# crisbodnar/text-to-image

Measured on AMD Instinct MI355X. Metric: images/sec (G+D step) at 64x64 batch=64, higher is better.
Workload: dtype f32; 1 GPU; wgancls 64x64 batch=64/GPU fp32, synthetic images + random 1024-d text embeddings, D step (+kt) then G step, Adam(b1=0,b2=0.9); global_batch=64, parallelism=dp1, launch=hipGraph replay (1 graph/iteration)

## Files before the change

text-to-image_amd/csrc/t2i_bgemm.hip:

```cpp
#include <hip/hip_runtime.h>
#include <stdint.h>

#include <type_traits>

#include "t2i_internal.h"

namespace t2i {

typedef float f32x16 __attribute__((ext_vector_type(16)));
typedef unsigned int u32x4 __attribute__((ext_vector_type(4)));

namespace {
constexpr int BK = 32;
constexpr int KSTRIDE = BK + 4;
constexpr unsigned OOB = 0xFFFFFFF0u;

template <int LAY, int WM, int WN, int NW = 4>
struct BSmem {
  static constexpr bool A_KIN = LAY != 2, B_KIN = LAY == 1;
  static constexpr int BM = 32 * (NW / 2) * WM, BN = 64 * WN;
  static constexpr int A_ELEMS = A_KIN ? BM * KSTRIDE : BK * BM;
  static constexpr int B_ELEMS = B_KIN ? BN * KSTRIDE : BK * BN;
  static constexpr int BYTES = 2 * (A_ELEMS + B_ELEMS) * 4;
};
// ... 86 lines not shown
      }
    }
  };

  float4 areg[A_LD], breg[B_LD];
  auto load_into = [&](float4* ar, float4* br) __attribute__((always_inline)) {
    const int k0 = l_t * BK;
    ++l_t;
#pragma unroll
    for (int i = 0; i < A_LD; ++i) {
      if (A_KIN) ar[i] = bl4(ra, a_off[i] + k0, a_ok[i] & (k0 + kq * 4 < p.K));
      else ar[i] = bl4(ra, a_off[i] + k0 * p.M, a_ok[i] & (k0 + a_kr + A_KR * i < p.K));
    }
#pragma unroll
    for (int i = 0; i < B_LD; ++i) {
      if (B_KIN) br[i] = bl4(rb, b_off[i] + k0, b_ok[i] & (k0 + kq * 4 < p.K));
      else br[i] = bl4(rb, b_off[i] + k0 * p.N, b_ok[i] & (k0 + b_kr + B_KR * i < p.K));
    }
  };
  auto load_tile = [&]() __attribute__((always_inline)) { load_into(areg, breg); };
  auto store_from = [&](int buf, const float4* ar, const float4* br) __attribute__((always_inline)) {
    float* as = As + buf * S::A_ELEMS;
    float* bs = Bs + buf * S::B_ELEMS;
#pragma unroll
    for (int i = 0; i < A_LD; ++i) {
      if (A_KIN) *reinterpret_cast<float4*>(&as[(r0 + RPP * i) * KSTRIDE + kq * 4]) = ar[i];
      else *reinterpret_cast<float4*>(&as[(a_kr + A_KR * i) * BM + a_c4 * 4]) = ar[i];
    }
#pragma unroll
    for (int i = 0; i < B_LD; ++i) {
      if (B_KIN) *reinterpret_cast<float4*>(&bs[(r0 + RPP * i) * KSTRIDE + kq * 4]) = br[i];
      else *reinterpret_cast<float4*>(&bs[(b_kr + B_KR * i) * BN + b_c4 * 4]) = br[i];
    }
  };
  auto store_tile = [&](int buf) __attribute__((always_inline)) { store_from(buf, areg, breg); };

  struct Frag { float a[WM][4]; float b[WN][4]; };
  auto read_frag = [&](Frag& f, const float* as, const float* bs, int c) __attribute__((always_inline)) {
#pragma unroll
    for (int i = 0; i < WM; ++i) {
      const int row = (wm * WM + i) * 32 + l31;
      if (A_KIN) {
        const float4 v = *reinterpret_cast<const float4*>(&as[row * KSTRIDE + c * 8 + lh * 4]);
        f.a[i][0] = v.x; f.a[i][1] = v.y; f.a[i][2] = v.z; f.a[i][3] = v.w;
      } else {
#pragma unroll
        for (int j = 0; j < 4; ++j) f.a[i][j] = as[(c * 8 + j + 4 * lh) * BM + row];
      }
    }
#pragma unroll
    for (int i = 0; i < WN; ++i) {
      const int col = (wn * WN + i) * 32 + l31;
      if (B_KIN) {
        const float4 v = *reinterpret_cast<const float4*>(&bs[col * KSTRIDE + c * 8 + lh * 4]);
        f.b[i][0] = v.x; f.b[i][1] = v.y; f.b[i][2] = v.z; f.b[i][3] = v.w;
      } else {
#pragma unroll
        for (int j = 0; j < 4; ++j) f.b[i][j] = bs[(c * 8 + j + 4 * lh) * BN + col];
      }
    }
  };

  f32x16 acc[WM][WN];
#pragma unroll
  for (int i = 0; i < WM; ++i)
#pragma unroll
    for (int n = 0; n < WN; ++n)
#pragma unroll
      for (int e = 0; e < 16; ++e) acc[i][n][e] = 0.f;
  auto mma_frag = [&](const Frag& f) __attribute__((always_inline)) {
#pragma unroll
    for (int j = 0; j < 4; ++j)
#pragma unroll
      for (int i = 0; i < WM; ++i)
#pragma unroll
        for (int n = 0; n < WN; ++n)
          acc[i][n] = __builtin_amdgcn_mfma_f32_32x32x2f32(f.a[i][j], f.b[n][j], acc[i][n], 0, 0, 0);
  };
  constexpr int N_MMA = 4 * WM * WN, N_PIECE = A_LD + B_LD, MMA_PER_PIECE = N_MMA / N_PIECE > 0 ? N_MMA / N_PIECE : 1;

  auto k_tile = [&](int t, Frag& c0, Frag& c1, Frag& n0, Frag& n1) __attribute__((always_inline)) {
    const float* as = As + (t & 1) * S::A_ELEMS;
    const float* bs = Bs + (t & 1) * S::B_ELEMS;
    const float* an = As + ((t + 1) & 1) * S::A_ELEMS;
    const float* bn_ = Bs + ((t + 1) & 1) * S::B_ELEMS;
    __builtin_amdgcn_sched_barrier(0);
    mma_frag(c0);
    __builtin_amdgcn_sched_barrier(0);
    read_frag(c0, as, bs, 2);
    __builtin_amdgcn_sched_barrier(0);
    mma_frag(c1);
    store_tile((t + 1) & 1);
#pragma unroll
    for (int q2 = 0; q2 < N_PIECE; ++q2) {
      __builtin_amdgcn_sched_group_barrier(0x008, MMA_PER_PIECE, 0);
      __builtin_amdgcn_sched_group_barrier(0x200, 1, 0);
    }
    __builtin_amdgcn_sched_barrier(0);
    read_frag(c1, as, bs, 3);
    __builtin_amdgcn_sched_barrier(0);
    __syncthreads();
    read_frag(n0, an, bn_, 0);
    read_frag(n1, an, bn_, 1);
    __builtin_amdgcn_sched_barrier(0);
    load_tile();
    mma_frag(c0);
#pragma unroll
    for (int q2 = 0; q2 < N_PIECE; ++q2) {
      __builtin_amdgcn_sched_group_barrier(0x008, MMA_PER_PIECE, 0);
      __builtin_amdgcn_sched_group_barrier(0x020, 1, 0);
    }
    __builtin_amdgcn_sched_barrier(0);
    mma_frag(c1);
  };

  next_item();
  {
    float4 a0[A_LD], b0[B_LD];
    load_into(a0, b0);
    load_tile();
    store_from(0, a0, b0);
  }
  __syncthreads();
  Frag fa0, fa1, fb0, fb1;
  read_frag(fa0, As, Bs, 0);
  read_frag(fa1, As, Bs, 1);
  for (int it = 0; it < n_items; ++it) {
    for (int t = 0; t < p.ntiles; t += 2) {
      if (t + 2 == p.ntiles) next_item();
      k_tile(0, fa0, fa1, fb0, fb1);
      k_tile(1, fb0, fb1, fa0, fa1);
    }
    int bz, bm, bn;
    coords(run0 + slot + it * nslot, bz, bm, bn);
    float* out = p.c + (int64_t)bz * p.sc;
#pragma unroll
    for (int i = 0; i < WM; ++i)
#pragma unroll
      for (int j = 0; j < WN; ++j) {
        const int n = bn + (wn * WN + j) * 32 + l31;
#pragma unroll
        for (int e = 0; e < 16; ++e) {
          const int m = bm + (wm * WM + i) * 32 + (e & 3) + 8 * (e >> 2) + 4 * lh;
          if (m < p.M && n < p.N) out[(size_t)m * p.N + n] = acc[i][j][e];
        }
#pragma unroll
        for (int e = 0; e < 16; ++e) acc[i][j][e] = 0.f;
      }
  }
}

template <int LAY, bool XF = false>
__global__ __launch_bounds__(256, 2) void bgemm9_kernel(Bgemm9Params q) {
  static_assert(!XF || LAY == 1, "the in-loader input transform exists for the input-gradient form");
  const BgemmParams& p = q.g;
  using S = BSmem<LAY, 1, 1, 4>;
  constexpr bool B_KIN = S::B_KIN;
  constexpr int BM = 64, BN = 64, A_LD = 2, B_LD = 2;
  constexpr int B_C4 = BN / 4, B_KR = 256 / B_C4;
  extern __shared__ __attribute__((aligned(16))) float smem_b[];
  float* As = smem_b;
  float* Bs = smem_b + 2 * S::A_ELEMS;

  const int tid = threadIdx.x;
  const int lane = tid & 63, wave = tid >> 6;
  const int wm = wave >> 1, wn = wave & 1;
  const int l31 = lane & 31, lh = lane >> 5;

  const int nslot = gridDim.x >> 3;
  const int xcd = blockIdx.x & 7, slot = blockIdx.x >> 3;
  const int qq = p.items >> 3, rr_ = p.items & 7;
  const int run0 = xcd * qq + min(xcd, rr_), runlen = qq + (xcd < rr_ ? 1 : 0);
  if (slot >= runlen) return;
  const int n_items = (runlen - slot + nslot - 1) / nslot;
  const int tiles = p.tiles_m * p.tiles_n;

  auto coords = [&](int w, int& phs, int& bm, int& bn) __attribute__((always_inline)) {
    phs = w / tiles;
    const int t = w - phs * tiles;
    const int g = p.group_n, per_group = g * p.tiles_m;
    const int grp = t / per_group, rr = t - grp * per_group, n0 = grp * g;
    const int width = min(g, p.tiles_n - n0);
    const int tm = rr / width;
    bm = tm * BM;
    bn = (n0 + rr - tm * width) * BN;
  };
  auto plane_slot = [&](int pos, int phs) __attribute__((always_inline)) {
    if (LAY == 0) return pos;
    const int r = pos / 3, c = pos - 3 * r;
    return ((2 - r) * 3 + (2 - c)) * 4 + (3 - phs);
  };

  const int kq = tid & 7, r0 = tid >> 3;
  const int b_c4 = tid % B_C4, b_kr = tid / B_C4;
  __amdgpu_buffer_rsrc_t ra, rb;
  int a_off[A_LD], b_off[B_LD];
  bool a_ok[A_LD], b_ok[B_LD];
  unsigned a_win[A_LD];
  int x_tap[4];
  unsigned x_bit[4];
  int l_item = -1, l_pos = 8, l_t = 0, l_phs = 0, l_bm = 0, l_bn = 0;
  if (XF) ra = __builtin_amdgcn_make_buffer_rsrc(const_cast<float*>(q.dy), (short)0, (int)p.a_bytes, 0x00020000);

  auto next_sub = [&]() __attribute__((always_inline)) {
    l_t = 0;
    bool new_item = false;
    if (++l_pos == 9) {
      l_pos = 0;
      ++l_item;
      new_item = true;
      if (l_item < n_items) coords(run0 + slot + l_item * nslot, l_phs, l_bm, l_bn);
    }
    if (l_item >= n_items) {
#pragma unroll
      for (int i = 0; i < A_LD; ++i) { a_ok[i] = false; a_win[i] = 0u; }
#pragma unroll
      for (int i = 0; i < B_LD; ++i) b_ok[i] = false;
      return;
    }
    const int ps = plane_slot(l_pos, l_phs);
    if (!XF) ra = __builtin_amdgcn_make_buffer_rsrc(const_cast<float*>(p.a + (int64_t)ps * p.sa), (short)0, (int)p.a_bytes, 0x00020000);
    rb = __builtin_amdgcn_make_buffer_rsrc(const_cast<float*>(p.b + (int64_t)ps * p.sb), (short)0, (int)p.b_bytes, 0x00020000);
    if (XF) {
      const int r = l_pos / 3, c = l_pos - 3 * r;
      const int rowpx = q.dWo * p.K;
      x_tap[0] = r * rowpx + c * p.K;  x_bit[0] = 1u << (r * 3 + c);
      x_tap[1] = 1 * rowpx + c * p.K;  x_bit[1] = r != 1 ? 1u << (3 + c) : 0u;
      x_tap[2] = r * rowpx + 1 * p.K;  x_bit[2] = c != 1 ? 1u << (r * 3 + 1) : 0u;
      x_tap[3] = 1 * rowpx + 1 * p.K;  x_bit[3] = (r != 1 && c != 1) ? 1u << 4 : 0u;
      if (new_item) {
        const int ph = l_phs >> 1, pw = l_phs & 1;
#pragma unroll
        for (int i = 0; i < A_LD; ++i) {
          const int m = l_bm + r0 + 32 * i;
          const int b = m / (q.Th * q.Tw), rem = m - b * (q.Th * q.Tw);
          const int ty = rem / q.Tw, tx = rem - ty * q.Tw;
          const int oh0 = 2 * ty + ph - 1, ow0 = 2 * tx + pw - 1;
          a_off[i] = ((b * q.dHo + oh0) * q.dWo + ow0) * p.K + kq * 4;
          unsigned w = 0u;
#pragma unroll
          for (int rr2 = 0; rr2 < 3; ++rr2)
#pragma unroll
            for (int cc2 = 0; cc2 < 3; ++cc2)
              if ((unsigned)(oh0 + rr2) < (unsigned)q.dHo && (unsigned)(ow0 + cc2) < (unsigned)q.dWo) w |= 1u << (rr2 * 3 + cc2);
          a_win[i] = m < p.M ? w : 0u;
        }
      }
    } else {
#pragma unroll
      for (int i = 0; i < A_LD; ++i) {
        const int m = l_bm + r0 + 32 * i;
        a_ok[i] = m < p.M;
        a_off[i] = m * p.K + kq * 4;
      }
    }
#pragma unroll
    for (int i = 0; i < B_LD; ++i) {
      if (B_KIN) {
        const int n = l_bn + r0 + 32 * i;
        b_ok[i] = n < p.N;
        b_off[i] = n * p.K + kq * 4;
      } else {
        const int n = l_bn + b_c4 * 4;
        b_ok[i] = n < p.N;
        b_off[i] = (b_kr + B_KR * i) * p.N + n;
      }
    }
  };

  float4 areg[A_LD], breg[B_LD];
  auto load_into = [&](float4* ar, float4* br) __attribute__((always_inline)) {
    const int k0 = l_t * BK;
    ++l_t;
    if (XF) {
      const bool kin = k0 + kq * 4 < p.K;
#pragma unroll
      for (int i = 0; i < A_LD; ++i) {
        const float4 ta = bl4(ra, a_off[i] + x_tap[0] + k0, kin & ((a_win[i] & x_bit[0]) != 0u));
        const float4 tb = bl4(ra, a_off[i] + x_tap[1] + k0, kin & ((a_win[i] & x_bit[1]) != 0u));
        const float4 tc = bl4(ra, a_off[i] + x_tap[2] + k0, kin & ((a_win[i] & x_bit[2]) != 0u));
        const float4 td = bl4(ra, a_off[i] + x_tap[3] + k0, kin & ((a_win[i] & x_bit[3]) != 0u));
        ar[i] = make_float4((ta.x - tb.x) - (tc.x - td.x), (ta.y - tb.y) - (tc.y - td.y), (ta.z - tb.z) - (tc.z - td.z), (ta.w - tb.w) - (tc.w - td.w));
      }
    } else {
#pragma unroll
      for (int i = 0; i < A_LD; ++i) ar[i] = bl4(ra, a_off[i] + k0, a_ok[i] & (k0 + kq * 4 < p.K));
    }
#pragma unroll
    for (int i = 0; i < B_LD; ++i) {
      if (B_KIN) br[i] = bl4(rb, b_off[i] + k0, b_ok[i] & (k0 + kq * 4 < p.K));
      else br[i] = bl4(rb, b_off[i] + k0 * p.N, b_ok[i] & (k0 + b_kr + B_KR * i < p.K));
    }
  };
  auto store_from = [&](int buf, const float4* ar, const float4* br) __attribute__((always_inline)) {
    float* as = As + buf * S::A_ELEMS;
    float* bs = Bs + buf * S::B_ELEMS;
#pragma unroll
    for (int i = 0; i < A_LD; ++i) *reinterpret_cast<float4*>(&as[(r0 + 32 * i) * KSTRIDE + kq * 4]) = ar[i];
#pragma unroll
    for (int i = 0; i < B_LD; ++i) {
      if (B_KIN) *reinterpret_cast<float4*>(&bs[(r0 + 32 * i) * KSTRIDE + kq * 4]) = br[i];
      else *reinterpret_cast<float4*>(&bs[(b_kr + B_KR * i) * BN + b_c4 * 4]) = br[i];
    }
  };

  struct Frag { float a[4]; float b[4]; };
  auto read_frag = [&](Frag& f, const float* as, const float* bs, int c) __attribute__((always_inline)) {
    {
      const int row = wm * 32 + l31;
      const float4 v = *reinterpret_cast<const float4*>(&as[row * KSTRIDE + c * 8 + lh * 4]);
      f.a[0] = v.x; f.a[1] = v.y; f.a[2] = v.z; f.a[3] = v.w;
    }
    {
      const int col = wn * 32 + l31;
      if (B_KIN) {
        const float4 v = *reinterpret_cast<const float4*>(&bs[col * KSTRIDE + c * 8 + lh * 4]);
        f.b[0] = v.x; f.b[1] = v.y; f.b[2] = v.z; f.b[3] = v.w;
      } else {
#pragma unroll
        for (int j = 0; j < 4; ++j) f.b[j] = bs[(c * 8 + j + 4 * lh) * BN + col];
      }
    }
  };

  f32x16 acc[9];
#pragma unroll
  for (int i = 0; i < 9; ++i)
#pragma unroll
    for (int e = 0; e < 16; ++e) acc[i][e] = 0.f;

  auto k_tile = [&](auto P_, int t, Frag& c0, Frag& c1, Frag& n0, Frag& n1) __attribute__((always_inline)) {
    constexpr int P = decltype(P_)::value;
    const float* as = As + (t & 1) * S::A_ELEMS;
    const float* bs = Bs + (t & 1) * S::B_ELEMS;
    const float* an = As + ((t + 1) & 1) * S::A_ELEMS;
    const float* bn_ = Bs + ((t + 1) & 1) * S::B_ELEMS;
    auto mma = [&](const Frag& f) __attribute__((always_inline)) {
#pragma unroll
      for (int j = 0; j < 4; ++j) acc[P] = __builtin_amdgcn_mfma_f32_32x32x2f32(f.a[j], f.b[j], acc[P], 0, 0, 0);
    };
    __builtin_amdgcn_sched_barrier(0);
    mma(c0);
    __builtin_amdgcn_sched_barrier(0);
    read_frag(c0, as, bs, 2);
    __builtin_amdgcn_sched_barrier(0);
    mma(c1);
    store_from((t + 1) & 1, areg, breg);
#pragma unroll
    for (int q2 = 0; q2 < 4; ++q2) {
      __builtin_amdgcn_sched_group_barrier(0x008, 1, 0);
      __builtin_amdgcn_sched_group_barrier(0x200, 1, 0);
    }
    __builtin_amdgcn_sched_barrier(0);
    read_frag(c1, as, bs, 3);
    __builtin_amdgcn_sched_barrier(0);
    __syncthreads();
    read_frag(n0, an, bn_, 0);
    read_frag(n1, an, bn_, 1);
    __builtin_amdgcn_sched_barrier(0);
    load_into(areg, breg);
    mma(c0);
#pragma unroll
    for (int q2 = 0; q2 < 4; ++q2) {
      __builtin_amdgcn_sched_group_barrier(0x008, 1, 0);
      __builtin_amdgcn_sched_group_barrier(0x020, 1, 0);
    }
    __builtin_amdgcn_sched_barrier(0);
    mma(c1);
  };

  next_sub();
  {
    float4 a0[A_LD], b0[B_LD];
    load_into(a0, b0);
    load_into(areg, breg);
    store_from(0, a0, b0);
  }
  __syncthreads();
  Frag fa0, fa1, fb0, fb1;
  read_frag(fa0, As, Bs, 0);
  read_frag(fa1, As, Bs, 1);
  auto run_pos = [&](auto P_) __attribute__((always_inline)) {
    for (int t = 0; t < p.ntiles; t += 2) {
      if (t + 2 == p.ntiles) next_sub();
      k_tile(P_, 0, fa0, fa1, fb0, fb1);
      k_tile(P_, 1, fb0, fb1, fa0, fa1);
    }
  };
  const int plane_px = q.Th * q.Tw;
  for (int it = 0; it < n_items; ++it) {
    run_pos(std::integral_constant<int, 0>{}); run_pos(std::integral_constant<int, 1>{}); run_pos(std::integral_constant<int, 2>{});
    run_pos(std::integral_constant<int, 3>{}); run_pos(std::integral_constant<int, 4>{}); run_pos(std::integral_constant<int, 5>{});
    run_pos(std::integral_constant<int, 6>{}); run_pos(std::integral_constant<int, 7>{}); run_pos(std::integral_constant<int, 8>{});
    int phs, bm, bn;
    coords(run0 + slot + it * nslot, phs, bm, bn);
    const int ph = phs >> 1, pw = phs & 1;
    const int n = bn + wn * 32 + l31;
    const float bs_ = (q.bias && n < p.N) ? q.bias[n] : 0.f;
#pragma unroll
    for (int e = 0; e < 16; ++e) {
      const int m = bm + wm * 32 + (e & 3) + 8 * (e >> 2) + 4 * lh;
      float z[2][3];
#pragma unroll
      for (int c = 0; c < 3; ++c) {
        z[0][c] = acc[0 * 3 + c][e] + acc[1 * 3 + c][e];
        z[1][c] = acc[1 * 3 + c][e] + acc[2 * 3 + c][e];
      }
      if (m < p.M && n < p.N) {
        const int b = m / plane_px, rem = m - b * plane_px;
        const int ty = rem / q.Tw, tx = rem - ty * q.Tw;
#pragma unroll
        for (int r = 0; r < 2; ++r) {
          const float y0 = apply_act((z[r][0] + z[r][1]) + bs_, q.act, q.alpha);
          const float y1 = apply_act((z[r][1] + z[r][2]) + bs_, q.act, q.alpha);
          const size_t oh = (size_t)q.sr * (2 * ty + r) + ph, ow0 = (size_t)q.sr * (2 * tx) + pw;
          float* o = q.out + (((size_t)b * q.OH + oh) * q.OW + ow0) * p.N + n;
          o[0] = y0;
          o[(size_t)q.sr * p.N] = y1;
        }
      }
    }
#pragma unroll
    for (int i = 0; i < 9; ++i)
#pragma unroll
      for (int e = 0; e < 16; ++e) acc[i][e] = 0.f;
  }
}

hipError_t bgemm9_launch(int lay, const Bgemm9Params& q, hipStream_t stream) {
  if (lay != 0 && lay != 1) return hipErrorInvalidValue;
  const int bytes = lay == 0 ? BSmem<0, 1, 1, 4>::BYTES : BSmem<1, 1, 1, 4>::BYTES;
  const int per_xcd = (q.g.items + 7) / 8;
  int nslot = per_xcd < 32 * 2 ? per_xcd : 32 * 2;
  if (nslot < 1) nslot = 1;
  if (lay == 0) hipLaunchKernelGGL((bgemm9_kernel<0, false>), dim3(nslot * 8), dim3(256), bytes, stream, q);
  else if (q.dy) hipLaunchKernelGGL((bgemm9_kernel<1, true>), dim3(nslot * 8), dim3(256), bytes, stream, q);
  else hipLaunchKernelGGL((bgemm9_kernel<1, false>), dim3(nslot * 8), dim3(256), bytes, stream, q);
  return hipGetLastError();
}

template <int LAY, int WM, int WN, int NW = 4>
static hipError_t launch_b(const BgemmParams& p, hipStream_t stream) {
  using S = BSmem<LAY, WM, WN, NW>;
  auto k = bgemm_kernel<LAY, WM, WN, NW>;
  static bool attr_done = false;
  if (!attr_done && S::BYTES > 48 * 1024) {
    hipError_t e = hipFuncSetAttribute(reinterpret_cast<const void*>(k), hipFuncAttributeMaxDynamicSharedMemorySize, S::BYTES);
    if (e != hipSuccess) return e;
    attr_done = true;
  }
  const int per_cu = (WM * WN == 1 && NW == 4) ? 4 : 2;
  const int per_xcd = (p.items + 7) / 8;
  int nslot = per_xcd < 32 * per_cu ? per_xcd : 32 * per_cu;
  if (nslot < 1) nslot = 1;
  hipLaunchKernelGGL(k, dim3(nslot * 8), dim3(64 * NW), S::BYTES, stream, p);
  return hipGetLastError();
}

hipError_t bgemm_launch(int lay, int wm, int wn, const BgemmParams& p, hipStream_t stream) {
  if (wm == 4 && wn == 1) {
    if (lay == 0) return launch_b<0, 1, 1, 8>(p, stream);
    if (lay == 1) return launch_b<1, 1, 1, 8>(p, stream);
    if (lay == 2) return launch_b<2, 1, 1, 8>(p, stream);
  }
#define T2I_B(L, a, b) if (lay == L && wm == a && wn == b) return launch_b<L, a, b>(p, stream);
  T2I_B(0, 1, 1) T2I_B(0, 2, 1) T2I_B(0, 1, 2) T2I_B(0, 2, 2)
  T2I_B(1, 1, 1) T2I_B(1, 2, 1) T2I_B(1, 1, 2) T2I_B(1, 2, 2)
  T2I_B(2, 1, 1) T2I_B(2, 2, 1) T2I_B(2, 1, 2) T2I_B(2, 2, 2)
#undef T2I_B
  return hipErrorInvalidValue;
}

}
```

text-to-image_amd/csrc/t2i_winograd.hip:

```cpp
#include <hip/hip_runtime.h>
#include <stdint.h>
#include <stdio.h>
#include <string.h>
#include <stdlib.h>

#include <mutex>
#include <vector>

#include "t2i_internal.h"

namespace t2i {

struct FilterEntry {
  const float* w; int kind, Cin, Cout; float* U; size_t bytes; unsigned long long cap; hipStream_t stream; bool valid;
  hipStream_t cap_fill = nullptr;
};
static std::mutex g_fc_mu;
static std::vector<FilterEntry> g_fc;
static int g_fc_on = 0;
static char* g_fc_buf = nullptr;
static size_t g_fc_cap = 0, g_fc_used = 0;

int filter_cache_attach(void* buf, size_t bytes) {
  std::lock_guard<std::mutex> lk(g_fc_mu);
// ... 327 lines not shown
  float* V = reinterpret_cast<float*>(base);
  float* Z = reinterpret_cast<float*>(base + al256(16 * T * d.Cin * 4));
  float* P = reinterpret_cast<float*>(base + al256(16 * T * d.Cin * 4) + al256(16 * T * d.Cout * 4));
  const int Th = d.H / 2, Tw = d.W / 2;
  if (Vhave) {
    V = const_cast<float*>(Vhave);
    if (valid_rows < d.B) {
      const size_t t0 = (size_t)valid_rows * Th * Tw, Tr = T - t0;
      hipLaunchKernelGGL(wino_input_kernel, dim3(wino_blocks(Tr * (d.Cin / 4))), dim3(256), 0, stream, x + (size_t)valid_rows * d.H * d.W * d.Cin, d.H,
                         d.W, d.Cin, Th, Tw, Tr, V + t0 * d.Cin, 0, Tp);
    }
  } else hipLaunchKernelGGL(wino_input_kernel, dim3(wino_blocks(T * (d.Cin / 4))), dim3(256), 0, stream, x, d.H, d.W, d.Cin, Th, Tw, T, V, 0, T);
  hipLaunchKernelGGL(wino_dy_kernel, dim3(wino_blocks(T * (d.Cout / 4))), dim3(256), 0, stream, dy, d.H, d.W, d.Cout, Th, Tw, T, Z);
  t2i_conv_desc gd = d;
  gd.B = (int32_t)T; gd.H = gd.W = gd.Ho = gd.Wo = 1; gd.KH = gd.KW = gd.SH = gd.SW = 1; gd.pad_t = gd.pad_l = 0;
  const int rc = run_batched_gemm(gd, MODE_BWD_FILTER, 16, V, Z, P, (int64_t)Tp * d.Cin, (int64_t)T * d.Cout, (int64_t)d.Cin * d.Cout, stream,
                                  "winograd filter-gradient gemm");
  if (rc != T2I_OK) return rc;
  hipLaunchKernelGGL(wino_dw_kernel, dim3(wino_blocks((size_t)d.Cin * (d.Cout / 4))), dim3(256), 0, stream, P, d.Cin, d.Cout, accumulate, dw);
  const hipError_t e = hipGetLastError();
  if (e != hipSuccess) { set_error("winograd filter gradient: %s", hipGetErrorString(e)); return T2I_ERR_LAUNCH; }
  return T2I_OK;
}

__device__ __forceinline__ void wino2_filter_body(const float* __restrict__ w, int Cin, int Cout, float* __restrict__ U, unsigned vb, unsigned nvb) {
  const int N4 = Cout >> 2;
  const size_t total = (size_t)4 * Cin * N4;
  const size_t plane = (size_t)4 * Cin * N4;
  for (size_t i = (size_t)vb * 256 + threadIdx.x; i < total; i += (size_t)nvb * 256) {
    const int n4 = (int)(i % N4);
    const int ci = (int)((i / N4) % Cin);
    const int ph = (int)(i / ((size_t)N4 * Cin));
    const int p = ph >> 1, q = ph & 1;
    float4 g[2][2];
#pragma unroll
    for (int a = 0; a < 2; ++a)
#pragma unroll
      for (int b = 0; b < 2; ++b)
        g[a][b] = reinterpret_cast<const float4*>(w + ((size_t)((2 * a + p) * 4 + (2 * b + q)) * Cin + ci) * Cout)[n4];
    float4 s[3][2] = {{g[0][0], g[0][1]}, {f4add(g[0][0], g[1][0]), f4add(g[0][1], g[1][1])}, {g[1][0], g[1][1]}};
    float4* o = reinterpret_cast<float4*>(U) + ((size_t)ph * Cin + ci) * N4 + n4;
#pragma unroll
    for (int r = 0; r < 3; ++r) {
      wst(&o[(size_t)(r * 3 + 0) * plane], s[r][0]);
      wst(&o[(size_t)(r * 3 + 1) * plane], f4add(s[r][0], s[r][1]));
      wst(&o[(size_t)(r * 3 + 2) * plane], s[r][1]);
    }
  }
}

__global__ __launch_bounds__(256) void wino2_filter_kernel(const float* __restrict__ w, int Cin, int Cout, float* __restrict__ U) {
  wino2_filter_body(w, Cin, Cout, U, blockIdx.x, gridDim.x);
}

__global__ __launch_bounds__(256) void wino2_input_kernel(const float* __restrict__ x, int H, int W, int C, int Th, int Tw, size_t T,
                                                          float* __restrict__ V, size_t plane_T) {
  const int C4 = C >> 2;
  const size_t total = T * 4 * C4;
  const size_t plane = plane_T * 4 * C4;
  for (size_t i = (size_t)blockIdx.x * blockDim.x + threadIdx.x; i < total; i += (size_t)gridDim.x * blockDim.x) {
    const int c4 = (int)(i % C4);
    const int ph = (int)((i / C4) & 3);
    const size_t t = i / ((size_t)4 * C4);
    const int p = ph >> 1, q = ph & 1;
    const int tx = (int)(t % Tw);
    const int ty = (int)((t / Tw) % Th);
    const size_t b = t / ((size_t)Tw * Th);
    float4 d[3][3];
#pragma unroll
    for (int r = 0; r < 3; ++r) {
      const int ih = 4 * ty - 1 + 2 * r + p;
#pragma unroll
      for (int c = 0; c < 3; ++c) {
        const int iw = 4 * tx - 1 + 2 * c + q;
        d[r][c] = ((unsigned)ih < (unsigned)H && (unsigned)iw < (unsigned)W)
                      ? reinterpret_cast<const float4*>(x + ((b * H + ih) * W + iw) * C)[c4]
                      : make_float4(0.f, 0.f, 0.f, 0.f);
      }
    }
    float4 tt[3][3];
#pragma unroll
    for (int c = 0; c < 3; ++c) {
      tt[0][c] = f4sub(d[0][c], d[1][c]);
      tt[1][c] = d[1][c];
      tt[2][c] = f4sub(d[2][c], d[1][c]);
    }
    float4* o = reinterpret_cast<float4*>(V) + (t * 4 + ph) * C4 + c4;
#pragma unroll
    for (int r = 0; r < 3; ++r) {
      wst(&o[(size_t)(r * 3 + 0) * plane], f4sub(tt[r][0], tt[r][1]));
      wst(&o[(size_t)(r * 3 + 1) * plane], tt[r][1]);
      wst(&o[(size_t)(r * 3 + 2) * plane], f4sub(tt[r][2], tt[r][1]));
    }
  }
}

__global__ __launch_bounds__(256) void wino2_output_kernel(const float* __restrict__ Mx, const float* __restrict__ bias, int Ho, int Wo,
                                                           int N, int Th, int Tw, size_t T, int act, float alpha,
                                                           float* __restrict__ y) {
  const int N4 = N >> 2;
  const size_t total = T * N4, plane = T * N4;
  for (size_t i = (size_t)blockIdx.x * blockDim.x + threadIdx.x; i < total; i += (size_t)gridDim.x * blockDim.x) {
    const int n4 = (int)(i % N4);
    const size_t t = i / N4;
    const int tx = (int)(t % Tw);
    const int ty = (int)((t / Tw) % Th);
    const size_t b = t / ((size_t)Tw * Th);
    const float4* m = reinterpret_cast<const float4*>(Mx) + t * N4 + n4;
    float4 z[2][3];
#pragma unroll
    for (int c = 0; c < 3; ++c) {
      const float4 m0 = m[(size_t)(0 * 3 + c) * plane], m1 = m[(size_t)(1 * 3 + c) * plane], m2 = m[(size_t)(2 * 3 + c) * plane];
      z[0][c] = f4add(m0, m1);
      z[1][c] = f4add(m1, m2);
    }
    const float4 bs = bias ? reinterpret_cast<const float4*>(bias)[n4] : make_float4(0.f, 0.f, 0.f, 0.f);
#pragma unroll
    for (int r = 0; r < 2; ++r) {
      float4 y0 = f4add(f4add(z[r][0], z[r][1]), bs);
      float4 y1 = f4add(f4add(z[r][1], z[r][2]), bs);
      y0.x = apply_act(y0.x, act, alpha); y0.y = apply_act(y0.y, act, alpha); y0.z = apply_act(y0.z, act, alpha); y0.w = apply_act(y0.w, act, alpha);
      y1.x = apply_act(y1.x, act, alpha); y1.y = apply_act(y1.y, act, alpha); y1.z = apply_act(y1.z, act, alpha); y1.w = apply_act(y1.w, act, alpha);
      float4* o = reinterpret_cast<float4*>(y + ((b * Ho + 2 * ty + r) * Wo + 2 * tx) * N) + n4;
      o[0] = y0;
      o[N4] = y1;
    }
  }
}

bool winograd_k4s2_eligible(const t2i_conv_desc& d, bool bwd_data) {
  const int minc = tuning().winograd_k4s2_minc;
  if (!tuning().winograd_k4s2 || d.math != T2I_MATH_F32) return false;
  if (!(d.KH == 4 && d.KW == 4 && d.SH == 2 && d.SW == 2 && d.pad_t == 1 && d.pad_l == 1)) return false;
  if ((d.H & 3) || (d.W & 3) || d.Ho * 2 != d.H || d.Wo * 2 != d.W) return false;
  if (bwd_data ? ((d.Cout % 32) || (d.Cin % 32)) : ((d.Cin % 8) || (d.Cout % 32))) return false;
  const int minc_bwd = tuning().winograd_k4s2_bwd_minc;
  const int m = bwd_data ? minc_bwd : minc;
  if (!(d.Cin >= m && d.Cout >= m)) return false;
  const int64_t T = (int64_t)d.B * (d.Ho / 2) * (d.Wo / 2);
  const int64_t items = 9 * ((T + 63) / 64) * ((d.Cout + 63) / 64);
  return T * 4 * d.Cin * d.Cout >= (int64_t)tuning().winograd_k4s2_minwork && items >= tuning().winograd_k4s2_minitems;
}

size_t winograd_k4s2_ws(const t2i_conv_desc& d) {
  const size_t T = (size_t)d.B * (d.Ho / 2) * (d.Wo / 2), K = (size_t)4 * d.Cin;
  return al256(9 * K * d.Cout * 4) + al256(9 * T * K * 4) + al256(9 * T * d.Cout * 4);
}

static int wino2_fused_gemm(int lay, int phases, size_t T, int N, int K, const float* V, const float* U, int64_t sa, int64_t sb, const float* bias,
                            float* out, int OH, int OW, int Th, int Tw, int sr, int act, float alpha, hipStream_t stream, const char* what,
                            const float* dy_raw = nullptr, int dHo = 0, int dWo = 0, int64_t dy_elems = 0) {
  const int mode = tuning().wino_fuse;
  if (!mode || !tuning().bgemm) return -1;
  const int ntiles = (K + 31) / 32;
  const int64_t a_elems = dy_raw ? dy_elems : (int64_t)T * K, b_elems = (int64_t)N * K;
  if (dy_raw) V = dy_raw;
  if ((ntiles & 1) || (T & 3) || (N & 3) || (K & 3) || (reinterpret_cast<uintptr_t>(V) & 15) || (reinterpret_cast<uintptr_t>(U) & 15) || (sa & 3) || (sb & 3) ||
      a_elems >= (1LL << 30) || b_elems >= (1LL << 30) || T >= (1u << 30))
    return -1;
  Bgemm9Params q;
  memset(&q, 0, sizeof(q));
  q.g.a = V; q.g.b = U; q.g.c = nullptr;
  q.g.M = (int32_t)T; q.g.N = N; q.g.K = K;
  q.g.tiles_m = (int32_t)((T + 63) / 64); q.g.tiles_n = (N + 63) / 64;
  { const int g = tuning().group_n; q.g.group_n = q.g.tiles_n < g ? q.g.tiles_n : g; if (q.g.group_n < 1) q.g.group_n = 1; }
  q.g.ntiles = ntiles;
  const int64_t items = (int64_t)phases * q.g.tiles_m * q.g.tiles_n;
  if (items >= (1LL << 30)) return -1;
  if (mode == 1) {
    const int64_t rounds = (items + 511) / 512;
    if (items < (int64_t)tuning().wino_fuse_items * (lay == 0 ? 4 : 1) || items * 100 < rounds * 512 * 85) return -1;
    if (K >= 1024 && rounds < 3) return -1;
  }
  q.g.items = (int32_t)items;
  q.g.sa = sa; q.g.sb = sb; q.g.sc = 0;
  q.g.a_bytes = (uint32_t)(a_elems * 4); q.g.b_bytes = (uint32_t)(b_elems * 4);
  q.bias = bias; q.out = out; q.OH = OH; q.OW = OW; q.Th = Th; q.Tw = Tw; q.sr = sr; q.act = act; q.alpha = alpha;
  q.dy = dy_raw; q.dHo = dHo; q.dWo = dWo;
  if (tuning().debug_plan) fprintf(stderr, "[t2i plan] %s: fused 9-position items, %d phases x %d x %d tiles, K=%d\n", what, phases, q.g.tiles_m, q.g.tiles_n, K);
  const hipError_t e = bgemm9_launch(lay, q, stream);
  if (e != hipSuccess) { set_error("%s: %s", what, hipGetErrorString(e)); return T2I_ERR_LAUNCH; }
  return T2I_OK;
}

int winograd_k4s2_fwd(const t2i_conv_desc& d, const float* x, const float* w, const float* bias, float* y, int act, float alpha,
                      void* ws, size_t ws_bytes, hipStream_t stream, float* Vkeep) {
  const size_t T = (size_t)d.B * (d.Ho / 2) * (d.Wo / 2), K = (size_t)4 * d.Cin;
  if (!ws || ws_bytes < winograd_k4s2_ws(d) || (reinterpret_cast<uintptr_t>(ws) & 15)) {
    set_error("winograd k4s2 conv: workspace %zu B < %zu B required (or misaligned)", ws_bytes, winograd_k4s2_ws(d));
    return T2I_ERR_WORKSPACE;
  }
  char* base = reinterpret_cast<char*>(ws);
  float* U = reinterpret_cast<float*>(base);
  float* V = Vkeep ? Vkeep : reinterpret_cast<float*>(base + al256(9 * K * d.Cout * 4));
  float* Mx = reinterpret_cast<float*>(base + al256(9 * K * d.Cout * 4) + al256(9 * T * K * 4));
  const int Th = d.Ho / 2, Tw = d.Wo / 2;
  bool fill = true;
  if (float* Uc = filter_cache_get(w, 2, d.Cin, d.Cout, (size_t)9 * 4 * d.Cin * d.Cout * 4, stream, &fill)) U = Uc;
  if (fill)
    hipLaunchKernelGGL(wino2_filter_kernel, dim3(wino_blocks((size_t)4 * d.Cin * (d.Cout / 4))), dim3(256), 0, stream, w, d.Cin, d.Cout, U);
  hipLaunchKernelGGL(wino2_input_kernel, dim3(wino_blocks(T * d.Cin)), dim3(256), 0, stream, x, d.H, d.W, d.Cin, Th, Tw, T, V, T);
  t2i_conv_desc gd = d;
  gd.B = (int32_t)T; gd.H = gd.W = gd.Ho = gd.Wo = 1; gd.Cin = (int32_t)K; gd.KH = gd.KW = gd.SH = gd.SW = 1; gd.pad_t = gd.pad_l = 0;
  {
    const int fr = wino2_fused_gemm(0, 1, T, d.Cout, (int)K, V, U, (int64_t)T * K, (int64_t)K * d.Cout, bias, y, d.Ho, d.Wo, Th, Tw, 1, act, alpha, stream,
                                    "winograd k4s2 fused gemm");
    if (fr != -1) return fr;
  }
  const int rc = run_batched_gemm(gd, MODE_FWD, 9, V, U, Mx, (int64_t)T * K, (int64_t)K * d.Cout, (int64_t)T * d.Cout, stream, "winograd k4s2 gemm");
  if (rc != T2I_OK) return rc;
  hipLaunchKernelGGL(wino2_output_kernel, dim3(wino_blocks(T * (d.Cout / 4))), dim3(256), 0, stream, Mx, bias, d.Ho, d.Wo, d.Cout, Th, Tw, T, act,
                     alpha, y);
  const hipError_t e = hipGetLastError();
  if (e != hipSuccess) { set_error("winograd k4s2 conv: %s", hipGetErrorString(e)); return T2I_ERR_LAUNCH; }
  return T2I_OK;
}

__device__ __forceinline__ int wino2b_slot(int r, int c, int phs) { return ((2 - r) * 3 + (2 - c)) * 4 + (3 - phs); }

__global__ __launch_bounds__(256) void wino2b_input_kernel(const float* __restrict__ dy, int Ho, int Wo, int C, int Th, int Tw, size_t T,
                                                           float* __restrict__ V) {
  const int C4 = C >> 2;
  const size_t total = T * 4 * C4;
  const size_t plane = T * C4;
  for (size_t i = (size_t)blockIdx.x * blockDim.x + threadIdx.x; i < total; i += (size_t)gridDim.x * blockDim.x) {
    const int c4 = (int)(i % C4);
    const size_t t = (i / C4) % T;
    const int phs = (int)(i / ((size_t)C4 * T));
    const int ph = phs >> 1, pw = phs & 1;
    const int tx = (int)(t % Tw);
    const int ty = (int)((t / Tw) % Th);
    const size_t b = t / ((size_t)Tw * Th);
    float4 d[3][3];
#pragma unroll
    for (int r = 0; r < 3; ++r) {
      const int oh = 2 * ty + ph - 1 + r;
#pragma unroll
      for (int c = 0; c < 3; ++c) {
        const int ow = 2 * tx + pw - 1 + c;
        d[r][c] = ((unsigned)oh < (unsigned)Ho && (unsigned)ow < (unsigned)Wo)
                      ? reinterpret_cast<const float4*>(dy + ((b * Ho + oh) * Wo + ow) * C)[c4]
                      : make_float4(0.f, 0.f, 0.f, 0.f);
      }
    }
    float4 tt[3][3];
#pragma unroll
    for (int c = 0; c < 3; ++c) {
      tt[0][c] = f4sub(d[0][c], d[1][c]);
      tt[1][c] = d[1][c];
      tt[2][c] = f4sub(d[2][c], d[1][c]);
    }
    float4* o = reinterpret_cast<float4*>(V) + t * C4 + c4;
#pragma unroll
    for (int r = 0; r < 3; ++r) {
      wst(&o[(size_t)wino2b_slot(r, 0, phs) * plane], f4sub(tt[r][0], tt[r][1]));
      wst(&o[(size_t)wino2b_slot(r, 1, phs) * plane], tt[r][1]);
      wst(&o[(size_t)wino2b_slot(r, 2, phs) * plane], f4sub(tt[r][2], tt[r][1]));
    }
  }
}

__global__ __launch_bounds__(256) void wino2b_output_kernel(const float* __restrict__ Mx, const float* __restrict__ bias, int H, int W,
                                                            int N, int Th, int Tw, size_t T, int act, float alpha,
                                                            float* __restrict__ dx) {
  const int N4 = N >> 2;
  const size_t total = T * 4 * N4, plane = T * N4;
  for (size_t i = (size_t)blockIdx.x * blockDim.x + threadIdx.x; i < total; i += (size_t)gridDim.x * blockDim.x) {
    const int n4 = (int)(i % N4);
    const size_t t = (i / N4) % T;
    const int phs = (int)(i / ((size_t)N4 * T));
    const int ph = phs >> 1, pw = phs & 1;
    const int tx = (int)(t % Tw);
    const int ty = (int)((t / Tw) % Th);
    const size_t b = t / ((size_t)Tw * Th);
    const float4* m = reinterpret_cast<const float4*>(Mx) + t * N4 + n4;
    float4 z[2][3];
#pragma unroll
    for (int c = 0; c < 3; ++c) {
      const float4 m0 = m[(size_t)wino2b_slot(0, c, phs) * plane], m1 = m[(size_t)wino2b_slot(1, c, phs) * plane],
                   m2 = m[(size_t)wino2b_slot(2, c, phs) * plane];
      z[0][c] = f4add(m0, m1);
      z[1][c] = f4add(m1, m2);
    }
    const float4 bs = bias ? reinterpret_cast<const float4*>(bias)[n4] : make_float4(0.f, 0.f, 0.f, 0.f);
#pragma unroll
    for (int r = 0; r < 2; ++r) {
      float4 y0 = f4add(f4add(z[r][0], z[r][1]), bs);
      float4 y1 = f4add(f4add(z[r][1], z[r][2]), bs);
      y0.x = apply_act(y0.x, act, alpha); y0.y = apply_act(y0.y, act, alpha); y0.z = apply_act(y0.z, act, alpha); y0.w = apply_act(y0.w, act, alpha);
      y1.x = apply_act(y1.x, act, alpha); y1.y = apply_act(y1.y, act, alpha); y1.z = apply_act(y1.z, act, alpha); y1.w = apply_act(y1.w, act, alpha);
      const size_t ih = (size_t)2 * (2 * ty + r) + ph;
      float4* o0 = reinterpret_cast<float4*>(dx + ((b * H + ih) * W + (size_t)2 * (2 * tx) + pw) * N) + n4;
      float4* o1 = reinterpret_cast<float4*>(dx + ((b * H + ih) * W + (size_t)2 * (2 * tx + 1) + pw) * N) + n4;
      *o0 = y0;
      *o1 = y1;
    }
  }
}

size_t winograd_k4s2_bwd_ws(const t2i_conv_desc& d) {
  const size_t T = (size_t)d.B * (d.Ho / 2) * (d.Wo / 2);
  return al256((size_t)36 * d.Cin * d.Cout * 4) + al256(36 * T * d.Cout * 4) + al256(36 * T * d.Cin * 4);
}

int winograd_k4s2_bwd_data(const t2i_conv_desc& d, const float* dy, const float* w, const float* bias, float* dx, int act, float alpha,
                           void* ws, size_t ws_bytes, hipStream_t stream) {
  const size_t T = (size_t)d.B * (d.Ho / 2) * (d.Wo / 2);
  if (!ws || ws_bytes < winograd_k4s2_bwd_ws(d) || (reinterpret_cast<uintptr_t>(ws) & 15)) {
    set_error("winograd k4s2 input gradient: workspace %zu B < %zu B required (or misaligned)", ws_bytes, winograd_k4s2_bwd_ws(d));
    return T2I_ERR_WORKSPACE;
// ... 327 lines not shown
```

Before: 5096 images/sec.

## Specialise fused Winograd input-gradient bgemm9 to reuse input taps via LDS parking

Replaces the generic XF path of bgemm9_kernel with a dedicated specialisation for the input-gradient Winograd form. The old path issued four global loads per A element to build the input transform. The new one iterates the nine plane positions in a fixed order, loads each tap once, and parks odd-position taps and the centre tap in extra LDS so later positions can form their differences from them. It keeps nine accumulators so the output transform and bias/activation happen in the epilogue, and it adds hand scheduling barriers. It also pads ntiles to an even count and relaxes the T alignment check for this path. In exchange it uses more LDS per block and many more accumulator registers, which may reduce occupancy.

New measurement: 5231 images/sec (median of 6 runs). 1.03x the previous value.

```diff
diff --git a/text-to-image_amd/csrc/t2i_bgemm.hip b/text-to-image_amd/csrc/t2i_bgemm.hip
--- a/text-to-image_amd/csrc/t2i_bgemm.hip
+++ b/text-to-image_amd/csrc/t2i_bgemm.hip
@@ -262,7 +262,7 @@
 
 template <int LAY, bool XF = false>
 __global__ __launch_bounds__(256, 2) void bgemm9_kernel(Bgemm9Params q) {
-  static_assert(!XF || LAY == 1, "the in-loader input transform exists for the input-gradient form");
+  static_assert(!XF, "the in-loader input transform is the specialisation bgemm9_kernel<1, true> below");
   const BgemmParams& p = q.g;
   using S = BSmem<LAY, 1, 1, 4>;
   constexpr bool B_KIN = S::B_KIN;
@@ -306,63 +306,30 @@
   __amdgpu_buffer_rsrc_t ra, rb;
   int a_off[A_LD], b_off[B_LD];
   bool a_ok[A_LD], b_ok[B_LD];
-  unsigned a_win[A_LD];
-  int x_tap[4];
-  unsigned x_bit[4];
   int l_item = -1, l_pos = 8, l_t = 0, l_phs = 0, l_bm = 0, l_bn = 0;
-  if (XF) ra = __builtin_amdgcn_make_buffer_rsrc(const_cast<float*>(q.dy), (short)0, (int)p.a_bytes, 0x00020000);
 
   auto next_sub = [&]() __attribute__((always_inline)) {
     l_t = 0;
-    bool new_item = false;
     if (++l_pos == 9) {
       l_pos = 0;
       ++l_item;
-      new_item = true;
       if (l_item < n_items) coords(run0 + slot + l_item * nslot, l_phs, l_bm, l_bn);
     }
     if (l_item >= n_items) {
 #pragma unroll
-      for (int i = 0; i < A_LD; ++i) { a_ok[i] = false; a_win[i] = 0u; }
+      for (int i = 0; i < A_LD; ++i) a_ok[i] = false;
 #pragma unroll
       for (int i = 0; i < B_LD; ++i) b_ok[i] = false;
       return;
     }
     const int ps = plane_slot(l_pos, l_phs);
-    if (!XF) ra = __builtin_amdgcn_make_buffer_rsrc(const_cast<float*>(p.a + (int64_t)ps * p.sa), (short)0, (int)p.a_bytes, 0x00020000);
+    ra = __builtin_amdgcn_make_buffer_rsrc(const_cast<float*>(p.a + (int64_t)ps * p.sa), (short)0, (int)p.a_bytes, 0x00020000);
     rb = __builtin_amdgcn_make_buffer_rsrc(const_cast<float*>(p.b + (int64_t)ps * p.sb), (short)0, (int)p.b_bytes, 0x00020000);
-    if (XF) {
-      const int r = l_pos / 3, c = l_pos - 3 * r;
-      const int rowpx = q.dWo * p.K;
-      x_tap[0] = r * rowpx + c * p.K;  x_bit[0] = 1u << (r * 3 + c);
-      x_tap[1] = 1 * rowpx + c * p.K;  x_bit[1] = r != 1 ? 1u << (3 + c) : 0u;
-      x_tap[2] = r * rowpx + 1 * p.K;  x_bit[2] = c != 1 ? 1u << (r * 3 + 1) : 0u;
-      x_tap[3] = 1 * rowpx + 1 * p.K;  x_bit[3] = (r != 1 && c != 1) ? 1u << 4 : 0u;
-      if (new_item) {
-        const int ph = l_phs >> 1, pw = l_phs & 1;
-#pragma unroll
-        for (int i = 0; i < A_LD; ++i) {
-          const int m = l_bm + r0 + 32 * i;
-          const int b = m / (q.Th * q.Tw), rem = m - b * (q.Th * q.Tw);
-          const int ty = rem / q.Tw, tx = rem - ty * q.Tw;
-          const int oh0 = 2 * ty + ph - 1, ow0 = 2 * tx + pw - 1;
-          a_off[i] = ((b * q.dHo + oh0) * q.dWo + ow0) * p.K + kq * 4;
-          unsigned w = 0u;
-#pragma unroll
-          for (int rr2 = 0; rr2 < 3; ++rr2)
-#pragma unroll
-            for (int cc2 = 0; cc2 < 3; ++cc2)
-              if ((unsigned)(oh0 + rr2) < (unsigned)q.dHo && (unsigned)(ow0 + cc2) < (unsigned)q.dWo) w |= 1u << (rr2 * 3 + cc2);
-          a_win[i] = m < p.M ? w : 0u;
-        }
-      }
-    } else {
-#pragma unroll
-      for (int i = 0; i < A_LD; ++i) {
-        const int m = l_bm + r0 + 32 * i;
-        a_ok[i] = m < p.M;
-        a_off[i] = m * p.K + kq * 4;
-      }
+#pragma unroll
+    for (int i = 0; i < A_LD; ++i) {
+      const int m = l_bm + r0 + 32 * i;
+      a_ok[i] = m < p.M;
+      a_off[i] = m * p.K + kq * 4;
     }
 #pragma unroll
     for (int i = 0; i < B_LD; ++i) {
@@ -382,20 +349,8 @@
   auto load_into = [&](float4* ar, float4* br) __attribute__((always_inline)) {
     const int k0 = l_t * BK;
     ++l_t;
-    if (XF) {
-      const bool kin = k0 + kq * 4 < p.K;
-#pragma unroll
-      for (int i = 0; i < A_LD; ++i) {
-        const float4 ta = bl4(ra, a_off[i] + x_tap[0] + k0, kin & ((a_win[i] & x_bit[0]) != 0u));
-        const float4 tb = bl4(ra, a_off[i] + x_tap[1] + k0, kin & ((a_win[i] & x_bit[1]) != 0u));
-        const float4 tc = bl4(ra, a_off[i] + x_tap[2] + k0, kin & ((a_win[i] & x_bit[2]) != 0u));
-        const float4 td = bl4(ra, a_off[i] + x_tap[3] + k0, kin & ((a_win[i] & x_bit[3]) != 0u));
-        ar[i] = make_float4((ta.x - tb.x) - (tc.x - td.x), (ta.y - tb.y) - (tc.y - td.y), (ta.z - tb.z) - (tc.z - td.z), (ta.w - tb.w) - (tc.w - td.w));
-      }
-    } else {
-#pragma unroll
-      for (int i = 0; i < A_LD; ++i) ar[i] = bl4(ra, a_off[i] + k0, a_ok[i] & (k0 + kq * 4 < p.K));
-    }
+#pragma unroll
+    for (int i = 0; i < A_LD; ++i) ar[i] = bl4(ra, a_off[i] + k0, a_ok[i] & (k0 + kq * 4 < p.K));
 #pragma unroll
     for (int i = 0; i < B_LD; ++i) {
       if (B_KIN) br[i] = bl4(rb, b_off[i] + k0, b_ok[i] & (k0 + kq * 4 < p.K));
@@ -537,6 +492,254 @@
   }
 }
 
+namespace {
+__host__ __device__ constexpr int w9_pos(int i) {
+  return i == 0 ? 4 : i == 1 ? 1 : i == 2 ? 3 : i == 3 ? 0 : i == 4 ? 5 : i == 5 ? 2 : i == 6 ? 7 : i == 7 ? 6 : 8;
+}
+constexpr int W9_PARK_BYTES = 4 * 2 * 256 * 16;
+__device__ __forceinline__ float4 sub4(float4 a, float4 b) { return make_float4(a.x - b.x, a.y - b.y, a.z - b.z, a.w - b.w); }
+}
+
+template <>
+__global__ __launch_bounds__(256, 2) void bgemm9_kernel<1, true>(Bgemm9Params q) {
+  const BgemmParams& p = q.g;
+  using S = BSmem<1, 1, 1, 4>;
+  constexpr int BM = 64, BN = 64;
+  extern __shared__ __attribute__((aligned(16))) float smem_b[];
+  float* As = smem_b;
+  float* Bs = smem_b + 2 * S::A_ELEMS;
+
+  const int tid = threadIdx.x;
+  const int lane = tid & 63, wave = tid >> 6;
+  const int wm = wave >> 1, wn = wave & 1;
+  const int l31 = lane & 31, lh = lane >> 5;
+  float4* park = reinterpret_cast<float4*>(smem_b + 2 * (S::A_ELEMS + S::B_ELEMS)) + tid;
+
+  const int nslot = gridDim.x >> 3;
+  const int xcd = blockIdx.x & 7, slot = blockIdx.x >> 3;
+  const int qq = p.items >> 3, rr_ = p.items & 7;
+  const int run0 = xcd * qq + min(xcd, rr_), runlen = qq + (xcd < rr_ ? 1 : 0);
+  if (slot >= runlen) return;
+  const int n_items = (runlen - slot + nslot - 1) / nslot;
+  const int tiles = p.tiles_m * p.tiles_n;
+
+  auto coords = [&](int w, int& phs, int& bm, int& bn) __attribute__((always_inline)) {
+    phs = w / tiles;
+    const int t = w - phs * tiles;
+    const int g = p.group_n, per_group = g * p.tiles_m;
+    const int grp = t / per_group, rr = t - grp * per_group, n0 = grp * g;
+    const int width = min(g, p.tiles_n - n0);
+    const int tm = rr / width;
+    bm = tm * BM;
+    bn = (n0 + rr - tm * width) * BN;
+  };
+
+  const int kq = tid & 7, r0 = tid >> 3;
+  const __amdgpu_buffer_rsrc_t ra = __builtin_amdgcn_make_buffer_rsrc(const_cast<float*>(q.dy), (short)0, (int)p.a_bytes, 0x00020000);
+  const int rowpx = q.dWo * p.K;
+  int a_off[2], b_off[2];
+  unsigned a_win[2];
+  bool b_ok[2];
+  int l_item = -1, l_t = p.ntiles - 1, l_phs = 0;
+
+  auto advance = [&]() __attribute__((always_inline)) {
+    if (++l_t < p.ntiles) return;
+    l_t = 0;
+    ++l_item;
+    if (l_item >= n_items) {
+#pragma unroll
+      for (int i = 0; i < 2; ++i) { a_win[i] = 0u; b_ok[i] = false; }
+      return;
+    }
+    int bm, bn;
+    coords(run0 + slot + l_item * nslot, l_phs, bm, bn);
+    const int ph = l_phs >> 1, pw = l_phs & 1;
+#pragma unroll
+    for (int i = 0; i < 2; ++i) {
+      const int m = bm + r0 + 32 * i;
+      const int b = m / (q.Th * q.Tw), rem = m - b * (q.Th * q.Tw);
+      const int ty = rem / q.Tw, tx = rem - ty * q.Tw;
+      const int oh0 = 2 * ty + ph - 1, ow0 = 2 * tx + pw - 1;
+      a_off[i] = ((b * q.dHo + oh0) * q.dWo + ow0) * p.K + kq * 4;
+      unsigned w = 0u;
+#pragma unroll
+      for (int rr2 = 0; rr2 < 3; ++rr2)
+#pragma unroll
+        for (int cc2 = 0; cc2 < 3; ++cc2)
+          if ((unsigned)(oh0 + rr2) < (unsigned)q.dHo && (unsigned)(ow0 + cc2) < (unsigned)q.dWo) w |= 1u << (rr2 * 3 + cc2);
+      a_win[i] = m < p.M ? w : 0u;
+      const int n = bn + r0 + 32 * i;
+      b_ok[i] = n < p.N;
+      b_off[i] = n * p.K + kq * 4;
+    }
+  };
+
+  float4 areg[2], breg[2];
+  auto load_stage = [&](auto I_, float4* ar, float4* br) __attribute__((always_inline)) {
+    constexpr int P = w9_pos(decltype(I_)::value), r = P / 3, c = P - 3 * r;
+    const int k0 = l_t * BK;
+    const bool kin = k0 + kq * 4 < p.K;
+    const int tap = r * rowpx + c * p.K + k0;
+#pragma unroll
+    for (int i = 0; i < 2; ++i) ar[i] = bl4(ra, a_off[i] + tap, kin & (((a_win[i] >> P) & 1u) != 0u));
+    const int ps = ((2 - r) * 3 + (2 - c)) * 4 + (3 - l_phs);
+    const __amdgpu_buffer_rsrc_t rb = __builtin_amdgcn_make_buffer_rsrc(const_cast<float*>(p.b + (int64_t)ps * p.sb), (short)0, (int)p.b_bytes, 0x00020000);
+#pragma unroll
+    for (int i = 0; i < 2; ++i) br[i] = bl4(rb, b_off[i] + k0, b_ok[i] & kin);
+  };
+
+  float4 c4[2];
+  auto park_read = [&](auto I_, float4* tb, float4* tc) __attribute__((always_inline)) {
+    constexpr int P = w9_pos(decltype(I_)::value), r = P / 3, c = P - 3 * r;
+    if (r != 1 && c != 1) {
+#pragma unroll
+      for (int i = 0; i < 2; ++i) {
+        tb[i] = park[(((3 + c) - 1) / 2 * 2 + i) * 256];
+        tc[i] = park[(((3 * r + 1) - 1) / 2 * 2 + i) * 256];
+      }
+    }
+  };
+  auto form_store = [&](auto I_, int buf, const float4* ar, const float4* br, const float4* pb, const float4* pc) __attribute__((always_inline)) {
+    constexpr int P = w9_pos(decltype(I_)::value), r = P / 3, c = P - 3 * r;
+    float* as = As + buf * S::A_ELEMS;
+    float* bs = Bs + buf * S::B_ELEMS;
+    const float4 zero = make_float4(0.f, 0.f, 0.f, 0.f);
+#pragma unroll
+    for (int i = 0; i < 2; ++i) *reinterpret_cast<float4*>(&bs[(r0 + 32 * i) * KSTRIDE + kq * 4]) = br[i];
+    if (P == 4) { c4[0] = ar[0]; c4[1] = ar[1]; }
+    if ((P & 1) != 0) {
+#pragma unroll
+      for (int i = 0; i < 2; ++i) park[((P - 1) / 2 * 2 + i) * 256] = ar[i];
+    }
+#pragma unroll
+    for (int i = 0; i < 2; ++i) {
+      const float4 tb = r == 1 ? zero : c == 1 ? c4[i] : pb[i];
+      const float4 tc = c == 1 ? zero : r == 1 ? c4[i] : pc[i];
+      const float4 td = (r != 1 && c != 1) ? c4[i] : zero;
+      *reinterpret_cast<float4*>(&as[(r0 + 32 * i) * KSTRIDE + kq * 4]) = sub4(sub4(ar[i], tb), sub4(tc, td));
+    }
+  };
+
+  struct Frag { float a[4]; float b[4]; };
+  auto read_frag = [&](Frag& f, const float* as, const float* bs, int c) __attribute__((always_inline)) {
+    const float4 va = *reinterpret_cast<const float4*>(&as[(wm * 32 + l31) * KSTRIDE + c * 8 + lh * 4]);
+    f.a[0] = va.x; f.a[1] = va.y; f.a[2] = va.z; f.a[3] = va.w;
+    const float4 vb = *reinterpret_cast<const float4*>(&bs[(wn * 32 + l31) * KSTRIDE + c * 8 + lh * 4]);
+    f.b[0] = vb.x; f.b[1] = vb.y; f.b[2] = vb.z; f.b[3] = vb.w;
+  };
+
+  f32x16 acc[9];
+#pragma unroll
+  for (int i = 0; i < 9; ++i)
+#pragma unroll
+    for (int e = 0; e < 16; ++e) acc[i][e] = 0.f;
+
+  auto k_tile = [&](auto I_, int t, Frag& c0, Frag& c1, Frag& n0, Frag& n1) __attribute__((always_inline)) {
+    constexpr int I = decltype(I_)::value, P = w9_pos(I);
+    using IN = std::integral_constant<int, (I + 1) % 9>;
+    using IL = std::integral_constant<int, (I + 2) % 9>;
+    const float* as = As + (t & 1) * S::A_ELEMS;
+    const float* bs = Bs + (t & 1) * S::B_ELEMS;
+    const float* an = As + ((t + 1) & 1) * S::A_ELEMS;
+    const float* bn_ = Bs + ((t + 1) & 1) * S::B_ELEMS;
+    auto mma = [&](const Frag& f) __attribute__((always_inline)) {
+#pragma unroll
+      for (int j = 0; j < 4; ++j) acc[P] = __builtin_amdgcn_mfma_f32_32x32x2f32(f.a[j], f.b[j], acc[P], 0, 0, 0);
+    };
+    float4 pb[2], pc[2];
+    __builtin_amdgcn_sched_barrier(0);
+    mma(c0);
+    __builtin_amdgcn_sched_barrier(0);
+    read_frag(c0, as, bs, 2);
+    park_read(IN{}, pb, pc);
+    __builtin_amdgcn_sched_barrier(0);
+    mma(c1);
+    form_store(IN{}, (t + 1) & 1, areg, breg, pb, pc);
+#pragma unroll
+    for (int q2 = 0; q2 < 4; ++q2) {
+      __builtin_amdgcn_sched_group_barrier(0x008, 1, 0);
+      __builtin_amdgcn_sched_group_barrier(0x002, 6, 0);
+      __builtin_amdgcn_sched_group_barrier(0x200, 2, 0);
+    }
+    __builtin_amdgcn_sched_barrier(0);
+    read_frag(c1, as, bs, 3);
+    __builtin_amdgcn_sched_barrier(0);
+    __syncthreads();
+    read_frag(n0, an, bn_, 0);
+    read_frag(n1, an, bn_, 1);
+    __builtin_amdgcn_sched_barrier(0);
+    load_stage(IL{}, areg, breg);
+    mma(c0);
+#pragma unroll
+    for (int q2 = 0; q2 < 4; ++q2) {
+      __builtin_amdgcn_sched_group_barrier(0x008, 1, 0);
+      __builtin_amdgcn_sched_group_barrier(0x020, 1, 0);
+    }
+    __builtin_amdgcn_sched_barrier(0);
+    mma(c1);
+  };
+
+  advance();
+  {
+    float4 a0[2], b0[2];
+    load_stage(std::integral_constant<int, 0>{}, a0, b0);
+    load_stage(std::integral_constant<int, 1>{}, areg, breg);
+    form_store(std::integral_constant<int, 0>{}, 0, a0, b0, a0, a0);
+  }
+  __syncthreads();
+  Frag fa0, fa1, fb0, fb1;
+  read_frag(fa0, As, Bs, 0);
+  read_frag(fa1, As, Bs, 1);
+#define T2I_W9_STAGE(I, u) \
+  if ((((u) + (I)) & 1) == 0) k_tile(std::integral_constant<int, I>{}, 0, fa0, fa1, fb0, fb1); \
+  else k_tile(std::integral_constant<int, I>{}, 1, fb0, fb1, fa0, fa1);
+#define T2I_W9_KTILE(u) \
+  T2I_W9_STAGE(0, u) T2I_W9_STAGE(1, u) T2I_W9_STAGE(2, u) T2I_W9_STAGE(3, u) T2I_W9_STAGE(4, u) T2I_W9_STAGE(5, u) T2I_W9_STAGE(6, u) \
+  advance(); \
+  T2I_W9_STAGE(7, u) T2I_W9_STAGE(8, u)
+  const int plane_px = q.Th * q.Tw;
+  for (int it = 0; it < n_items; ++it) {
+    for (int t = 0; t < p.ntiles; t += 2) {
+      T2I_W9_KTILE(0)
+      T2I_W9_KTILE(1)
+    }
+#undef T2I_W9_KTILE
+#undef T2I_W9_STAGE
+    int phs, bm, bn;
+    coords(run0 + slot + it * nslot, phs, bm, bn);
+    const int ph = phs >> 1, pw = phs & 1;
+    const int n = bn + wn * 32 + l31;
+    const float bs_ = (q.bias && n < p.N) ? q.bias[n] : 0.f;
+#pragma unroll
+    for (int e = 0; e < 16; ++e) {
+      const int m = bm + wm * 32 + (e & 3) + 8 * (e >> 2) + 4 * lh;
+      float z[2][3];
+#pragma unroll
+      for (int c = 0; c < 3; ++c) {
+        z[0][c] = acc[0 * 3 + c][e] + acc[1 * 3 + c][e];
+        z[1][c] = acc[1 * 3 + c][e] + acc[2 * 3 + c][e];
+      }
+      if (m < p.M && n < p.N) {
+        const int b = m / plane_px, rem = m - b * plane_px;
+        const int ty = rem / q.Tw, tx = rem - ty * q.Tw;
+#pragma unroll
+        for (int r = 0; r < 2; ++r) {
+          const float y0 = apply_act((z[r][0] + z[r][1]) + bs_, q.act, q.alpha);
+          const float y1 = apply_act((z[r][1] + z[r][2]) + bs_, q.act, q.alpha);
+          const size_t oh = (size_t)q.sr * (2 * ty + r) + ph, ow0 = (size_t)q.sr * (2 * tx) + pw;
+          float* o = q.out + (((size_t)b * q.OH + oh) * q.OW + ow0) * p.N + n;
+          o[0] = y0;
+          o[(size_t)q.sr * p.N] = y1;
+        }
+      }
+    }
+#pragma unroll
+    for (int i = 0; i < 9; ++i)
+#pragma unroll
+      for (int e = 0; e < 16; ++e) acc[i][e] = 0.f;
+  }
+}
+
 hipError_t bgemm9_launch(int lay, const Bgemm9Params& q, hipStream_t stream) {
   if (lay != 0 && lay != 1) return hipErrorInvalidValue;
   const int bytes = lay == 0 ? BSmem<0, 1, 1, 4>::BYTES : BSmem<1, 1, 1, 4>::BYTES;
@@ -544,8 +747,16 @@
   int nslot = per_xcd < 32 * 2 ? per_xcd : 32 * 2;
   if (nslot < 1) nslot = 1;
   if (lay == 0) hipLaunchKernelGGL((bgemm9_kernel<0, false>), dim3(nslot * 8), dim3(256), bytes, stream, q);
-  else if (q.dy) hipLaunchKernelGGL((bgemm9_kernel<1, true>), dim3(nslot * 8), dim3(256), bytes, stream, q);
-  else hipLaunchKernelGGL((bgemm9_kernel<1, false>), dim3(nslot * 8), dim3(256), bytes, stream, q);
+  else if (q.dy) {
+    constexpr int wbytes = BSmem<1, 1, 1, 4>::BYTES + W9_PARK_BYTES;
+    static bool attr_done = false;
+    if (!attr_done) {
+      hipError_t e = hipFuncSetAttribute(reinterpret_cast<const void*>(bgemm9_kernel<1, true>), hipFuncAttributeMaxDynamicSharedMemorySize, wbytes);
+      if (e != hipSuccess) return e;
+      attr_done = true;
+    }
+    hipLaunchKernelGGL((bgemm9_kernel<1, true>), dim3(nslot * 8), dim3(256), wbytes, stream, q);
+  } else hipLaunchKernelGGL((bgemm9_kernel<1, false>), dim3(nslot * 8), dim3(256), bytes, stream, q);
   return hipGetLastError();
 }
 
diff --git a/text-to-image_amd/csrc/t2i_winograd.hip b/text-to-image_amd/csrc/t2i_winograd.hip
--- a/text-to-image_amd/csrc/t2i_winograd.hip
+++ b/text-to-image_amd/csrc/t2i_winograd.hip
@@ -503,10 +503,10 @@
                             const float* dy_raw = nullptr, int dHo = 0, int dWo = 0, int64_t dy_elems = 0) {
   const int mode = tuning().wino_fuse;
   if (!mode || !tuning().bgemm) return -1;
-  const int ntiles = (K + 31) / 32;
+  const int ntiles = dy_raw ? ((K + 31) / 32 + 1) & ~1 : (K + 31) / 32;
   const int64_t a_elems = dy_raw ? dy_elems : (int64_t)T * K, b_elems = (int64_t)N * K;
   if (dy_raw) V = dy_raw;
-  if ((ntiles & 1) || (T & 3) || (N & 3) || (K & 3) || (reinterpret_cast<uintptr_t>(V) & 15) || (reinterpret_cast<uintptr_t>(U) & 15) || (sa & 3) || (sb & 3) ||
+  if ((ntiles & 1) || (!dy_raw && (T & 3)) || (N & 3) || (K & 3) || (reinterpret_cast<uintptr_t>(V) & 15) || (reinterpret_cast<uintptr_t>(U) & 15) || (sa & 3) || (sb & 3) ||
       a_elems >= (1LL << 30) || b_elems >= (1LL << 30) || T >= (1u << 30))
     return -1;
   Bgemm9Params q;
```
